# UBCMOCCA/mocca_envs

Hardware: AMD Instinct MI355X
Metric: env-steps/sec, Walker3DCustomEnv-v0 @ 4096 envs, 1/2/4/8 MI355X (higher is better)
Workload: dtype f32; 1 GPU; Walker3DCustomEnv-v0, 4096 envs/GPU, flat ground, U(-1,1) action tape, auto-reset; max_rows=48, max_contacts=12, envs_per_gpu=4096, parallelism=independent env shards x1, no collective, preroll_steps=6088

## Files before the change

### mocca_envs_amd/csrc/mocca_device.h

```cpp
#pragma once

#include <hip/hip_runtime.h>
#include <stdint.h>

#include "mocca_model.h"
#include "mocca_philox.h"
#include "topo_walker3d.h"
#include "topo_cassie.h"
#include "topo_walker2d.h"
#include "topo_crab2d.h"
#include "topo_laikago.h"

#define DI __device__ __forceinline__

#ifndef MOCCA_NS
#define MOCCA_NS mocca
#endif
#ifndef MOCCA_MAXR
#define MOCCA_MAXR 48
#endif
#ifndef MOCCA_COMPACT
#define MOCCA_COMPACT 0
#endif

// ... 82 lines not shown
  L_XL = L_V,
  L_MID = L_CAND + (MOCCA_MAX_PAIRS + 1) / 2,
  L_LGAP = L_GP,
  L_TOTAL = L_V + MAXR * MAXR + 28 + MOCCA_LDS_PAD,
#endif
};
static_assert(L_ABA_END <= L_TOTAL, "ABA view must fit");
static_assert(L_SV % 4 == 0 && SVS % 4 == 0 && SVS >= 16, "joint records live in the body records, 16-byte aligned");
static_assert(L_J + (MAXR + 1) * 28 <= L_TOTAL, "Jacobian rows (+ dummy) must fit the tail of the A region");
static_assert(L_J % 4 == 0 && L_V % 4 == 0 && L_RT % 4 == 0 && L_CT % 4 == 0, "16-byte alignment of broadcast rows");
static_assert(MAXR % 2 == 0 && 3 * MAXC <= MAXR, "friction rows sit on the top 2 MAXC lanes of the row range, odd lane = second tangent");
static_assert(L_PLANK + 12 * MOCCA_MAX_PLANKS <= L_V && L_Q0 + 16 <= L_V, "persistent region overflows into the two-view region");
#if MOCCA_COMPACT
static_assert(L_TOTAL * 4 <= 8192 || MOCCA_LDS_PAD > 0, "more than 8 KB of LDS per wave: fewer than 20 waves per CU (5 per SIMD)");
static_assert(L_J >= L_SV + 22 * SVS, "J rows are written while S, V, 1/D are still being read");
static_assert(L_CAND + (MOCCA_MAX_PAIRS + 1) / 2 <= L_ABA_END && L_RT + 264 <= L_GP, "frames, geom points and the candidate list live under the link inertias");
#else
static_assert(L_TOTAL * 4 <= 10240 || MOCCA_LDS_PAD > 0 || MAXR > 48, "more than 10 KB of LDS per wave: fewer than 16 waves per CU, the 4096-env batch no longer fits one round");
static_assert(MAXR != 48 || (L_ROWD == L_V + 848 && L_RT == L_V + 896 && L_M == L_V + 1160 && L_P == L_V + 1952 && L_ABA_END == L_V + 2084 && L_J == L_V + 960), "the product's layout is unchanged");
static_assert(COMPACT || L_CAND + (MOCCA_MAX_PAIRS + 1) / 2 <= L_TOTAL, "candidate list behind the ABA view");
static_assert(L_J >= L_RT, "J rows may be written while S, U, 1/D, the factor of IA0 and the contacts are still being read");
static_assert(L_LGAP + MAXR <= L_CT && L_J >= L_CT, "limit gaps: written after the collision pass, read before the first J row or A entry is stored");
#endif
#if MOCCA_COMPACT
static_assert(L_LGAP >= L_J + 28 * (MAXR + 1) && L_LGAP >= L_A + MAXR * MAXR && L_LGAP >= L_M && L_LGAP + MAXR <= L_TOTAL, "limit gaps: behind the solver view, in the dead link inertias");
#endif
static_assert(L_MID % 4 == 0 && L_MID >= L_CAND + (MOCCA_MAX_PAIRS + 1) / 2, "midpoint records: 16-byte aligned, behind the candidate list");
template <class T>
#ifdef MOCCA_NO_TRIM_1
constexpr bool MID_RECORDS = false;
#else
constexpr bool MID_RECORDS = T::NPAIR > 0 && 6 * T::NG <= GP_FLOATS && L_MID + 4 * T::NG <= (COMPACT ? (int)L_ABA_END : (int)L_TOTAL);
#endif

enum : int { C_BA = 0, C_BB = 1, C_SLOT = 2, C_P = 3, C_N = 6, C_DEPTH = 9, C_MU = 10, C_ERP = 11, C_CFM = 12, C_MA = 13, C_MB = 14 };

struct StepArgs {
  const MoccaModel* model;
  float* dyn;
  uint32_t* task;
  float* terrain;
  const float* act;
  float* obs;
  float* rew;
  uint8_t* done;
  int32_t* info;
  const uint8_t* mask;
  int n_envs;
  int obs_dim;
  int auto_reset;
  int eval_mode;
  int random_pose;
  int curriculum;
  int host_retarget;
  int env_offset;
  uint32_t seed_lo, seed_hi;
  const float* curriculum_v;
  const float* eval_mode_v;
  int random_reward;
  const float* gain_v;
  float gain;
  const int32_t* inj_touch;
  const int32_t* inj_target;
  const int32_t* inj_body;
  const float* tape;
  int tape_n;
  int32_t* dbg;
  const float* traj;
  int traj_n;
  double traj_tmax, traj_cstep;
  int prio;
  const float* hf;
  int hf_rows, hf_cols;
  float hf_scale;
  float* final_obs;
  int persist_warm;
  const int32_t* order;
  int pace;
  unsigned long long* pace_acc;
  float* ep_ret;
  float* ep_masks;
  float* ep_bad;
  void* ep_rec;
  float* ep_totals;
  uint32_t ep_serial;
  float* robot_state;
  const float* base_value;
  int32_t* hf_field;
  int hf_stride, hf_n_fields, hf_redraw;
};
constexpr int ROBOT_STATE_STRIDE = 64;

DI void wsync() {
  __builtin_amdgcn_fence(__ATOMIC_RELEASE, "wavefront");
  __builtin_amdgcn_wave_barrier();
  __builtin_amdgcn_fence(__ATOMIC_ACQUIRE, "wavefront");
}
DI float dot3(const float* a, const float* b) { return a[0] * b[0] + a[1] * b[1] + a[2] * b[2]; }
DI void cross3(const float* a, const float* b, float* o) {
  float x = a[1] * b[2] - a[2] * b[1], y = a[2] * b[0] - a[0] * b[2], z = a[0] * b[1] - a[1] * b[0];
  o[0] = x; o[1] = y; o[2] = z;
}
DI float dot6(const float* a, const float* b) {
  return a[0] * b[0] + a[1] * b[1] + a[2] * b[2] + a[3] * b[3] + a[4] * b[4] + a[5] * b[5];
}
DI void matvec3(const float* R, const float* x, float* o) {
  float a = R[0] * x[0] + R[1] * x[1] + R[2] * x[2];
  float b = R[3] * x[0] + R[4] * x[1] + R[5] * x[2];
  float c = R[6] * x[0] + R[7] * x[1] + R[8] * x[2];
  o[0] = a; o[1] = b; o[2] = c;
}
DI void matmul3(const float* A, const float* B, float* C) {
  float T[9];
#pragma unroll
  for (int i = 0; i < 3; ++i)
#pragma unroll
    for (int j = 0; j < 3; ++j) T[3 * i + j] = A[3 * i] * B[j] + A[3 * i + 1] * B[3 + j] + A[3 * i + 2] * B[6 + j];
#pragma unroll
  for (int i = 0; i < 9; ++i) C[i] = T[i];
}
DI void quat_to_mat(const float* q, float* R) {
  float x = q[0], y = q[1], z = q[2], w = q[3];
  R[0] = 1 - 2 * (y * y + z * z); R[1] = 2 * (x * y - z * w); R[2] = 2 * (x * z + y * w);
  R[3] = 2 * (x * y + z * w); R[4] = 1 - 2 * (x * x + z * z); R[5] = 2 * (y * z - x * w);
  R[6] = 2 * (x * z - y * w); R[7] = 2 * (y * z + x * w); R[8] = 1 - 2 * (x * x + y * y);
// ... 104 lines not shown
  v = fmaxf(v, dpp_mov<0x140>(v));
  return fmaxf(fmaxf(readlane(v, 0), readlane(v, 16)), fmaxf(readlane(v, 32), readlane(v, 48)));
}

DI float rng_uniform(uint32_t slo, uint32_t shi, uint32_t env, uint32_t episode, uint32_t d) {
  uint32_t o[4];
  philox4x32(d >> 2, episode, env, 0u, slo, shi, o);
  uint32_t w = (d & 3) == 0 ? o[0] : (d & 3) == 1 ? o[1] : (d & 3) == 2 ? o[2] : o[3];
  return (float)(w >> 8) * (1.0f / 16777216.0f);
}

template <bool INJECT>
DI float draw_u(const StepArgs& a, int env, int episode, int d) {
  if constexpr (INJECT) {
    if (a.tape) return d < a.tape_n ? a.tape[(size_t)(env - a.env_offset) * a.tape_n + d] : 0.5f;
  }
  return rng_uniform(a.seed_lo, a.seed_hi, (uint32_t)env, (uint32_t)episode, (uint32_t)d);
}

struct WalkConsts { float cl[3], inl[6], ms, jarm, jdamp; };
template <bool FULL>
DI void walk_consts(ModelP M, int b, WalkConsts& k) {
#pragma unroll
  for (int i = 0; i < 3; ++i) k.cl[i] = M->com[b][i];
#pragma unroll
  for (int i = 0; i < 6; ++i) k.inl[i] = 0.0f;
  k.ms = 0; k.jarm = 0; k.jdamp = 0;
  if (FULL) {
#pragma unroll
    for (int i = 0; i < 6; ++i) k.inl[i] = M->inertia[b][i];
    k.ms = M->mass[b]; k.jarm = M->jarm[b]; k.jdamp = M->jdamp[b];
  }
}
template <class T>
DI void walk_phase1(float* L, int lane, unsigned long long ppk) {
  static_assert(3 * (T::NB - 1) <= 63, "three lanes per body must fit the wave (lane 63 writes the base)");
  {
    const int g = (lane * 43) >> 7;
    const int ri = lane - 3 * g;
    const int bg = g + 1 < T::NB ? g + 1 : 0;
    const unsigned plo = (unsigned)__shfl((int)(unsigned)ppk, bg, 64), phi = (unsigned)__shfl((int)(unsigned)(ppk >> 32), bg, 64);
    const unsigned long long pk3 = ((unsigned long long)phi << 32) | plo;
    float Rb[9];
    {
      float q[4] = {L[L_BASE + 3], L[L_BASE + 4], L[L_BASE + 5], L[L_BASE + 6]};
      quat_to_mat(q, Rb);
    }
    float row[3] = {ri == 0 ? Rb[0] : ri == 1 ? Rb[3] : Rb[6], ri == 0 ? Rb[1] : ri == 1 ? Rb[4] : Rb[7], ri == 0 ? Rb[2] : ri == 1 ? Rb[5] : Rb[8]};
    float rr = 0.0f;
#pragma unroll
    for (int k = 0; k < T::MAXD; ++k) {
      const int j = (int)((pk3 >> (5 * k)) & 31ull);
      const float4* jr = reinterpret_cast<const float4*>(L + L_SV + SVS * j);
      const float4 r0 = jr[0], r1 = jr[1], r2 = jr[2];
      rr += row[0] * r2.y + row[1] * r2.z + row[2] * r2.w;
      const float n0 = row[0] * r0.x + row[1] * r0.w + row[2] * r1.z;
      const float n1 = row[0] * r0.y + row[1] * r1.x + row[2] * r1.w;
      const float n2 = row[0] * r0.z + row[1] * r1.y + row[2] * r2.x;
      row[0] = n0; row[1] = n1; row[2] = n2;
    }
    if (bg > 0) {
      const float4 r3 = reinterpret_cast<const float4*>(L + L_SV + SVS * bg)[3];
      *reinterpret_cast<float4*>(L + L_RT + 12 * bg + 4 * ri) = make_float4(row[0], row[1], row[2], rr);
      L[L_SV + SVS * bg + ri] = row[0] * r3.x + row[1] * r3.y + row[2] * r3.z;
    }
    if (lane == 63) {
#pragma unroll
      for (int i = 0; i < 3; ++i) *reinterpret_cast<float4*>(L + L_RT + 4 * i) = make_float4(Rb[3 * i], Rb[3 * i + 1], Rb[3 * i + 2], 0.0f);
    }
  }
}
template <class T, bool FULL>
DI void walk_phase2(ModelP M, float* L, int lane, int b, unsigned long long ppk, const WalkConsts& wk) {
  const float cl[3] = {wk.cl[0], wk.cl[1], wk.cl[2]};
  const float inl[6] = {wk.inl[0], wk.inl[1], wk.inl[2], wk.inl[3], wk.inl[4], wk.inl[5]};
  const float ms = wk.ms, jarm = wk.jarm, jdamp = wk.jdamp;
  float R[9], r[3], v[6], S[6] = {0, 0, 0, 0, 0, 0}, c[6] = {0, 0, 0, 0, 0, 0};
#pragma unroll
  for (int i = 0; i < 3; ++i) {
    const float4 t = *reinterpret_cast<const float4*>(L + L_RT + 12 * b + 4 * i);
    R[3 * i] = t.x; R[3 * i + 1] = t.y; R[3 * i + 2] = t.z; r[i] = t.w;
  }
  if (FULL) {
    if (lane >= 1 && lane < T::NB) {
      float a[3] = {L[L_SV + SVS * b], L[L_SV + SVS * b + 1], L[L_SV + SVS * b + 2]}, ra[3];
      cross3(r, a, ra);
#pragma unroll
      for (int i = 0; i < 3; ++i) { S[i] = a[i]; S[3 + i] = ra[i]; L[L_SV + SVS * b + 3 + i] = ra[i]; }
    }
    wsync();
#pragma unroll
    for (int k = 0; k < 3; ++k) { v[k] = L[L_BASE + 10 + k]; v[3 + k] = L[L_BASE + 7 + k]; }
#pragma unroll
    for (int k = 0; k < T::MAXD; ++k) {
      const int j = (int)((ppk >> (5 * k)) & 31ull);
      if (j != 0 && j != b) {
        const float qd = L[L_QD + j];
// ... 53 lines not shown
      p[0] -= cw[1] * fz; p[1] -= -cw[0] * fz; p[5] -= fz;
      {
        float om[3] = {v[0], v[1], v[2]}, Iom[3], wxc[3], F[3], cxF[3];
        float Iwf[9] = {Iw[0], Iw[1], Iw[2], Iw[1], Iw[4], Iw[5], Iw[2], Iw[5], Iw[8]};
        matvec3(Iwf, om, Iom);
        cross3(om, cw, wxc);
        float vc[3] = {v[3] + wxc[0], v[4] + wxc[1], v[5] + wxc[2]};
        const float kl = unif(M->lin_damp) * ms * (1.0f + __builtin_sqrtf(dot3(vc, vc)));
        const float ka = unif(M->ang_damp) * (1.0f + __builtin_sqrtf(dot3(om, om)));
#pragma unroll
        for (int i = 0; i < 3; ++i) F[i] = kl * vc[i];
        cross3(cw, F, cxF);
#pragma unroll
        for (int i = 0; i < 3; ++i) { p[i] += ka * Iom[i] + cxF[i]; p[3 + i] += F[i]; }
      }
#pragma unroll
      for (int i = 0; i < 6; ++i)
#pragma unroll
        for (int jx = 0; jx < 6; ++jx) L[L_M + 36 * b + 6 * i + jx] = I[sym(i, jx)];
#pragma unroll
      for (int i = 0; i < 6; ++i) L[L_P + 6 * b + i] = p[i];
      L[L_SV + SVS * b + SV_INVD] = jarm;
      L[L_SV + SVS * b + SV_UU] = L[L_TAU + b] - jdamp * L[L_QD + b];
    }
  }
}

template <class T, bool FULL>
DI void walk_kinematics(ModelP M, float* L, int lane, unsigned long long ppk) {
  asm volatile("" : "+v"(lane));
  const int b = lane < T::NB ? lane : 0;
  WalkConsts wk;
  walk_consts<FULL>(M, b, wk);
  walk_phase1<T>(L, lane, ppk);
  wsync();
  walk_phase2<T, FULL>(M, L, lane, b, ppk, wk);
}

DI void chol6_factor(const float* A, float* F) {
  float Lm[6][6];
#pragma unroll
  for (int j = 0; j < 6; ++j) {
    float s = A[sym(j, j)];
#pragma unroll
    for (int k = 0; k < j; ++k) s -= Lm[j][k] * Lm[j][k];
    const float id = rsq(s);
    F[sym(j, j)] = id;
#pragma unroll
    for (int i = j + 1; i < 6; ++i) {
      float t = A[sym(i, j)];
#pragma unroll
      for (int k = 0; k < j; ++k) t -= Lm[i][k] * Lm[j][k];
      Lm[i][j] = t * id;
      F[sym(i, j)] = Lm[i][j];
    }
  }
}
DI void chol6_solve(const float* F, const float* b, float* x) {
  float y[6];
#pragma unroll
  for (int j = 0; j < 6; ++j) {
    float t = b[j];
#pragma unroll
    for (int k = 0; k < j; ++k) t -= F[sym(j, k)] * y[k];
    y[j] = t * F[sym(j, j)];
  }
#pragma unroll
// ... 1172 lines not shown
    for (int i = 0; i < 6; ++i) { S[i] = L[L_SV + SVS * jj + i]; U[i] = L[L_SV + SVS * jj + SV_V + i]; }
    float jb = dot6(S, F);
    if (jj == jl) jb = sgn;
    jb = valid ? jb : 0.0f;
    const float uu = valid ? (k == T::MAXD - 1 ? jb : jb - dot6(S, pa)) : 0.0f;
#pragma unroll
    for (int i = 0; i < 6; ++i) pa[i] += U[i] * uu;
    if (valid) Jrow[5 + jj] = jb;
    w += jb * L[L_NU + 5 + jj];
    pu[k] = uu * L[L_SV + SVS * jj + SV_INVD];
    pin6(pa); pin1(pu[k]); pin1(w);
  }
  if (two_paths) {
    const int bq = bb >= 0 ? bb : 0;
    const unsigned long long pkb = ((unsigned long long)(unsigned)__shfl((int)(unsigned)(ppk >> 32), bq, 64) << 32) |
                                   (unsigned long long)(unsigned)__shfl((int)(unsigned)ppk, bq, 64);
#pragma unroll
    for (int k = T::MAXD - 1; k >= 0; --k) {
      const int j = (int)((pkb >> (5 * k)) & 31ull);
      const bool valid = j != 0;
      const int jj = j;
      float S[6], U[6];
#pragma unroll
      for (int i = 0; i < 6; ++i) { S[i] = L[L_SV + SVS * jj + i]; U[i] = L[L_SV + SVS * jj + SV_V + i]; }
      const float jb = valid ? -dot6(S, F2) : 0.0f;
      const float uu = valid ? (k == T::MAXD - 1 ? jb : jb - dot6(S, pb)) : 0.0f;
#pragma unroll
      for (int i = 0; i < 6; ++i) pb[i] += U[i] * uu;
      if (valid) Jrow[5 + jj] += jb;
      w += jb * L[L_NU + 5 + jj];
      pub[k] = uu * L[L_SV + SVS * jj + SV_INVD];
      pin6(pb); pin1(pub[k]); pin1(w);
    }
  } else {
#pragma unroll
    for (int k = 0; k < T::MAXD; ++k) pub[k] = 0.0f;
  }
  STAMP(19);
  int l2off = 0;
  asm volatile("" : "+v"(l2off));
  l2off &= ~3;
  const float* L2 = L + l2off;
  float a0[6];
  {
    float rhs[6];
#pragma unroll
    for (int i = 0; i < 6; ++i) {
      const float jb = F[i] * sa - F2[i] * sb;
      Jrow[i] = jb;
      w += jb * L[L_NU + i];
      rhs[i] = jb - (pa[i] + pb[i]);
    }
    chol6_solve(Afac, rhs, a0);
#pragma unroll
    for (int i = 0; i < 6; ++i) X[i] = a0[i];
  }
  {
    float acc[T::NB][6];
#pragma unroll
    for (int i = 0; i < 6; ++i) acc[0][i] = a0[i];
#pragma unroll
    for (int b = 1; b < T::NB; ++b) {
      const int p = T::parent(b);
      float S[6], U[6];
#pragma unroll
      for (int i = 0; i < 6; ++i) { S[i] = L2[L_SV + SVS * b + i]; U[i] = L2[L_SV + SVS * b + SV_V + i]; }
      const int dpos = T::depth(b) - 1;
      float ub = __uint_as_float(__float_as_uint(pu[dpos]) & (unsigned)__builtin_amdgcn_sbfe((int)ma, b, 1));
      if (two_paths) ub += __uint_as_float(__float_as_uint(pub[dpos]) & (unsigned)__builtin_amdgcn_sbfe((int)mb, b, 1));
      const float qdd = ub - dot6(U, acc[p]);
      X[5 + b] = qdd;
#pragma unroll
      for (int i = 0; i < 6; ++i) acc[b][i] = acc[p][i] + S[i] * qdd;
      pin6(acc[b]); pin1(X[5 + b]);
    }
  }
  STAMP(6);
  wsync();
  const int lc = has_row ? dense : MAXR - 1;
  float diag;
  bool on_mfma = false;
  if constexpr (T::NCLOS == 0 && MATRIX_PIPE) on_mfma = nr >= MOCCA_DELASSUS_MFMA_MIN && nr <= DELASSUS_MFMA_ROWS && !(wave_flags & 2);
  if (on_mfma) {
    diag = delassus_mfma<T>(L, X, has_row ? dense : 0, has_row, nr, lane);
  } else {
    float av[MAXR / 2 + 1];
    const int cc = has_row ? dense : 0, tmax = nr >> 1;
    delassus_dots<T, 0>(L, X, 28 * cc, 28 * nr, tmax, av);
    diag = has_row ? av[0] : 1.0f;
    wsync();
    if (has_row) delassus_store<0>(L, cc, nr, tmax, av);
  }
  const float invdiag = diag + cfm > 1e-12f ? rcp(diag + cfm) : 0.0f;
  wsync();
  STAMP(7);
  if (__ballot(lam != 0.0f) != 0ull) {
    int rr = nl + NFIX;
    const int rend = nl + NFIX + nc;
#pragma unroll 1
    for (; rr + 2 <= rend; rr += 2) {
      const float g0 = L[L_A + MAXR * rr + lc], g1 = L[L_A + MAXR * rr + MAXR + lc];
      w += g0 * readlane(lam, rr); w += g1 * readlane(lam, rr + 1);
    }
    if (rr < rend) w += L[L_A + MAXR * rr + lc] * readlane(lam, rr);
  }
  STAMP(20);
  const int iters = uni(M->n_iters);
// ... 108 lines not shown
      const float k = hdt * sinc;
      dq[0] = om[0] * k; dq[1] = om[1] * k; dq[2] = om[2] * k;
    } else {
      const float wn = sqrtf(dot3(om, om)), sn = sinf(wn * hdt) / wn;
      dq[0] = om[0] * sn; dq[1] = om[1] * sn; dq[2] = om[2] * sn; dq[3] = cosf(wn * hdt);
    }
    const float q0 = L[L_BASE + 3], q1 = L[L_BASE + 4], q2 = L[L_BASE + 5], q3 = L[L_BASE + 6];
    float nq[4];
    nq[0] = dq[3] * q0 + dq[0] * q3 + dq[1] * q2 - dq[2] * q1;
    nq[1] = dq[3] * q1 - dq[0] * q2 + dq[1] * q3 + dq[2] * q0;
    nq[2] = dq[3] * q2 + dq[0] * q1 - dq[1] * q0 + dq[2] * q3;
    nq[3] = dq[3] * q3 - dq[0] * q0 - dq[1] * q1 - dq[2] * q2;
    const float nn = rsq(nq[0] * nq[0] + nq[1] * nq[1] + nq[2] * nq[2] + nq[3] * nq[3]);
#pragma unroll
    for (int i = 0; i < 4; ++i) L[L_BASE + 3 + i] = nq[i] * nn;
  }
  wsync();
}

DI void fast_sincos(float q, float* s, float* c) {
  const float k = rintf(q * 0.636619772f);
  float r = fmaf(-k, 1.57079601e+00f, q);
  r = fmaf(-k, 3.13916473e-07f, r);
  r = fmaf(-k, 5.39030253e-15f, r);
  const float r2 = r * r;
  const float sr = r + r * r2 * (-1.0f / 6 + r2 * (1.0f / 120 + r2 * (-1.0f / 5040 + r2 * (1.0f / 362880))));
  const float cr = 1.0f + r2 * (-0.5f + r2 * (1.0f / 24 + r2 * (-1.0f / 720 + r2 * (1.0f / 40320 + r2 * (-1.0f / 3628800)))));
  const int qd = (int)k & 3;
  const float ss = (qd & 1) ? cr : sr, cc = (qd & 1) ? sr : cr;
  *s = (qd & 2) ? -ss : ss;
  *c = ((qd + 1) & 2) ? -cc : cc;
}

template <class T>
DI void stage_joints(ModelP M, float* L, int lane) {
  if (lane < T::NB) {
    const int j = lane;
    float s, cq;
    fast_sincos(L[L_Q + j], &s, &cq);
    const float t = 1.0f - cq;
    float ax[3], jr[9], Rq[9], Tl[9];
#pragma unroll
    for (int i = 0; i < 3; ++i) ax[i] = M->jaxis[j][i];
#pragma unroll
    for (int i = 0; i < 9; ++i) jr[i] = M->jrot[j][i];
    Rq[0] = cq + t * ax[0] * ax[0];          Rq[1] = t * ax[0] * ax[1] - s * ax[2];   Rq[2] = t * ax[0] * ax[2] + s * ax[1];
    Rq[3] = t * ax[0] * ax[1] + s * ax[2];   Rq[4] = cq + t * ax[1] * ax[1];          Rq[5] = t * ax[1] * ax[2] - s * ax[0];
    Rq[6] = t * ax[0] * ax[2] - s * ax[1];   Rq[7] = t * ax[1] * ax[2] + s * ax[0];   Rq[8] = cq + t * ax[2] * ax[2];
    matmul3(jr, Rq, Tl);
    float4* rec = reinterpret_cast<float4*>(L + L_SV + SVS * j);
    rec[0] = make_float4(Tl[0], Tl[1], Tl[2], Tl[3]);
    rec[1] = make_float4(Tl[4], Tl[5], Tl[6], Tl[7]);
    rec[2] = make_float4(Tl[8], M->jpos[j][0], M->jpos[j][1], M->jpos[j][2]);
    rec[3] = make_float4(ax[0], ax[1], ax[2], L[L_QD + j]);
  }
  wsync();
}

template <class T, int TASK>
DI ContactFlags substep(ModelP M, float* L, int lane, const float* ter, int next_step_index,
                        unsigned long long ppk, int32_t* dbg, int prio, int& rows_out,
                        const HeightFieldArgs hfa = HeightFieldArgs{nullptr, 0, 0, 0.0f}, int sidx = 0, int nsub = 1, int* cover_out = nullptr) {
  const int per0 = 64 + MOCCA_PACE_ROWUNIT * rows_out, done0 = sidx * per0, total = nsub * per0;
  STAMP(30);
  stage_joints<T>(M, L, lane);
  STAMP(29);
  int nc = 0, nc_wanted = 0;
  float Afac[21] = {0, 0, 0, 0, 0, 0, 0, 0, 0, 0, 0, 0, 0, 0, 0, 0, 0, 0, 0, 0, 0};
  ContactFlags fl = {0, 0, 0, 0, 0, 0, 0, 0, 0};
  if constexpr (COMPACT) {
    static_assert(!COMPACT || T::NCLOS == 0, "closure rows read the body frames after the ABA: not in the compact layout");
    int wl = lane;
    asm volatile("" : "+v"(wl));
    walk_phase1<T>(L, wl, ppk);
    wsync();
    STAMP(0);
    geom_points<T>(M, L, lane);
    wsync();
    STAMP(15);
#ifndef MOCCA_SKIP_COLLIDE
    fl = collide<T, TASK>(M, L, lane, ter, next_step_index, &nc, dbg, &nc_wanted, hfa, cover_out);
#endif
    wsync();
    const int wb = wl < T::NB ? wl : 0;
    WalkConsts wk;
    walk_consts<true>(M, wb, wk);
    walk_phase2<T, true>(M, L, wl, wb, ppk, wk);
// ... 226 lines not shown
      dx = sg * (mx < d1 ? mx : d1);
    }
    float x = 0, y = 0, z = 0, rx = 0, ry = 0, rz = 0;
#pragma unroll 1
    for (int k = 0; k < N; ++k) {
      rx += readlane(dx, k); ry += readlane(dy, k); rz += readlane(dz, k);
      if (lane == k) { x = rx; y = ry; z = rz; }
    }
    if (lane < N) {
      ter[6 * i] = x; ter[6 * i + 1] = y; ter[6 * i + 2] = z; ter[6 * i + 3] = phi; ter[6 * i + 4] = xt; ter[6 * i + 5] = yt;
    }
    if (lane == 0) { ter[120] = 0.0f; ter[121] = 1.0f; ter[122] = 2.0f; ter[123] = 3.0f; }
  }
  wsync();
}

DI int live_curriculum(const StepArgs& a, int env) {
  if (a.curriculum_v) { const int c = (int)a.curriculum_v[env]; return c < 0 ? 0 : (c > 9 ? 9 : c); }
  return a.curriculum;
}
DI bool live_eval_mode(const StepArgs& a, int env) { return a.eval_mode_v ? a.eval_mode_v[env] != 0.0f : a.eval_mode != 0; }

template <class T>
DI float reset_base_pose(ModelP M, float* L, int lane) {
  if (lane == 0) {
#pragma unroll
    for (int i = 0; i < 3; ++i) { L[L_BASE + i] = M->init_pos[i]; L[L_BASE + 7 + i] = M->init_vel[i]; L[L_BASE + 10 + i] = 0; }
#pragma unroll
    for (int i = 0; i < 4; ++i) L[L_BASE + 3 + i] = M->init_quat[i];
  }
  if (lane < MOCCA_MAX_SLOTS) L[L_WARM + lane] = 0.0f;
  wsync();
  const float z0 = L[L_BASE + 2];
  stage_joints<T>(M, L, lane);
  walk_kinematics<T, false>(M, L, lane, T::path_packed(lane < T::NB ? lane : 0));
  wsync();
  return z0;
}

template <class T, int TASK, bool INJECT = false>
DI void reset_env(const StepArgs& a, ModelP M, float* L, float* ter, int env, int lane, TaskRegs& t,
                  float* obs) {
  const int ep = t.episode + 1, cur = t.cur;
  const float sfc[4] = {t.fc0, t.fc1, t.fc2, t.fc3};
  const int snsi = t.nsi, scover = t.cover;
  t = TaskRegs{};
  t.episode = ep;
  if (TASK == MOCCA_TASK_WALKER3D_STEPPER && (M->task_flags & MOCCA_TASKF_STALE_RESET_CONTACTS)) {
    t.fc0 = sfc[0]; t.fc1 = sfc[1]; t.fc2 = sfc[2]; t.fc3 = sfc[3];
    const int npl = M->n_planks;
    int reached = cover_targets(scover, snsi, npl, 0) | cover_targets(scover, snsi, npl, 1);
    if constexpr (T::NFEET > 2) reached |= cover_targets(scover, snsi, npl, 2) | cover_targets(scover, snsi, npl, 3);
    if (reached) t.trc = 1;
  }
  t.cur = TASK == MOCCA_TASK_WALKER3D_STEPPER ? live_curriculum(a, env - a.env_offset) : cur;
  t.gain = a.gain_v ? a.gain_v[env - a.env_offset] : a.gain;
  if (TASK == MOCCA_TASK_WALKER3D_CUSTOM) {
    randomize_target<INJECT>(a, env, t, live_eval_mode(a, env - a.env_offset));
    float sa, ca;
    fast_sincos(t.angle, &sa, &ca);
    t.wt[0] = t.dist * ca;
    t.wt[1] = t.dist * sa;
    t.wt[2] = 1.0f;
  } else if (TASK == MOCCA_TASK_WALKER3D_STEPPER) {
    t.gain = M->gain_cur[0] + (M->gain_cur[1] - M->gain_cur[0]) * t.cur / 9;
  }
  t.mirrored = draw_u<INJECT>(a, env, t.episode, t.draw) < 0.5f;
// ... 237 lines not shown
```

### mocca_envs_amd/csrc/mocca_kernels.h

```cpp
#pragma once
#include <hip/hip_runtime.h>

#include "mocca.h"
#include "mocca_device.h"

namespace MOCCA_NS {

#ifndef MOCCA_WAVES_PER_EU
#define MOCCA_WAVES_PER_EU 4
#endif

DI void flush_obs(const float* L, float* dst, int lane, int obs_dim) {
#pragma unroll 1
  for (int k = lane; k < obs_dim; k += 64) dst[k] = L[L_OBS + k];
}
DI void keep_terminal_obs(const StepArgs& a, const float* L, int env, int lane) {
  wsync();
  if (a.final_obs) flush_obs(L, a.final_obs + (size_t)env * a.obs_dim, lane, a.obs_dim);
  wsync();
}

template <class T>
DI void keep_robot_state(const StepArgs& a, const float* L, int env, int lane) {
  static_assert(ROBOT_OBS<T> <= 64 && ROBOT_OBS<T> <= ROBOT_STATE_STRIDE, "one store per lane");
// ... 155 lines not shown
  if (cur_idx != t.nsi) calc_potential(M, L, t, ro, &dist, &cd, &sd);
  float rew;
  if (!a.random_reward) {
    rew = progress - energy + step_bonus + bonus + tall - posture - joints;
  } else {
    const float terms[8] = {progress, -energy, step_bonus, bonus, 0.0f, tall, -posture, -joints};
    rew = 0.0f;
#pragma unroll
    for (int k = 0; k < 8; ++k) {
      float w;
      if (a.random_reward == 1) {
        w = 0.8f + 0.4f * draw_u<INJECT>(a, env + a.env_offset, t.episode, t.draw + k);
        if (lane == 0) tk[MOCCA_TW_REWARD_WEIGHTS + k] = __float_as_uint(w);
      } else {
        w = __uint_as_float(tk[MOCCA_TW_REWARD_WEIGHTS + k]);
      }
      rew += w * terms[k];
    }
    if (a.random_reward == 1) t.draw += 8;
  }
  t.cover = cover;
  return {rew, t.nsi};
}

template <class T>
DI StepResult cassie_step(const StepArgs& __restrict__ a, ModelP M, float* L, uint32_t* tk, int lane, unsigned long long ppk, TaskRegs& __restrict__ t,
                          float* obs) {
  t.istep += M->n_llc;
  float jv = 0.0f;
  if (lane < M->n_ordered) {
    jv = (L[L_Q + M->ordered_body[lane]] - L[L_Q0 + lane]) / M->control_dt;
    tk[MOCCA_TW_JVEL + lane] = __float_as_uint(jv);
  }
  stage_joints<T>(M, L, lane);
  walk_kinematics<T, false>(M, L, lane, ppk);
  wsync();
  t.t += 1;
  const CassieState cs = cassie_state(M, L, lane, t.initz);
  const float old = t.linpot;
  t.linpot = cassie_potential(M, L);
  const float alive = cs.height > M->alive_height ? 2.0f : -1.0f;
  if (!cs.finite || alive < 0.0f) t.done = 1;
  float rew = alive + (t.linpot - old);
  float phase = 0.0f;
  if (M->cassie_mode != MOCCA_CASSIE_PLAIN) {
    const int f1 = traj_frame(a, M, t.istep, &phase);
    rew = cassie_mocap_reward(a, M, L, lane, cs, jv, f1);
  }
  cassie_observe(M, L, lane, cs, t.initz, jv, phase, obs);
  return {rew, 0};
}

template <class T, int TASK, bool INJECT = false>
__global__ __launch_bounds__(64, MOCCA_WAVES_PER_EU) void mocca_step_kernel(StepArgs a) {
  __shared__ float L[L_TOTAL];
  const int lane = threadIdx.x;
  if ((int)blockIdx.x >= a.n_envs) return;
  const int env = a.order ? uni(a.order[blockIdx.x]) : (int)blockIdx.x;
  ModelP M = (ModelP)a.model;
  float* st = a.dyn + (size_t)env * DYN_STRIDE;
  uint32_t* tk = a.task + (size_t)env * MOCCA_TASK_WORDS;
  float* ter = TASK == MOCCA_TASK_WALKER3D_STEPPER ? a.terrain + (size_t)env * TERRAIN_STRIDE : nullptr;
  float* obs_out = a.obs + (size_t)env * a.obs_dim;
  float* obs = L + L_OBS;
  int32_t* dbg = a.dbg ? a.dbg + (size_t)env * MOCCA_DEBUG_WORDS : nullptr;

  const bool warm_ld = INJECT || uni(__float_as_int(M->warmstart)) != 0, warm_st = warm_ld || a.persist_warm != 0;
  if (dbg && lane == 0) { dbg[16] = 0; dbg[17] = 0; dbg[18] = 0; }
  load_dyn(st, L, lane, T::NJ, T::NSLOT, warm_ld);
  pace_start(a, L, lane, INJECT ? 0 : a.pace);
  if (lane == 0) L[L_KEEPWARM] = __int_as_float((warm_st ? 1 : 0) | ((a.prio & PRIO_DELASSUS_VALU) ? 2 : 0));
  const unsigned long long ppk = T::path_packed(lane < T::NB ? lane : 0);
  ContactFlags fl = {0, 0, 0, 0, 0, 0, 0, 0, 0};
  int cover = 0;
  if constexpr (TASK == MOCCA_TASK_CASSIE) {
    const int no = M->n_ordered, nctl = M->n_ctrl, mode = M->cassie_mode;
    float target = 0.0f;
    if (lane < nctl) {
      float base = M->ctrl_base[lane];
      if (mode != MOCCA_CASSIE_PLAIN) {
        const int f0 = traj_frame(a, M, (int)tk[MOCCA_TW_ISTEP]);
        base = (lane < nctl - 2 && M->residual_control) ? a.traj[(size_t)f0 * MOCCA_TRAJ_STRIDE + M->ctrl_oidx[lane]] : 0.0f;
      }
      target = base + (lane < nctl - 2 ? a.act[(size_t)env * (nctl - 2) + lane] : 0.0f);
    }
    if (lane < no) {
      L[L_JVEL + lane] = __uint_as_float(tk[MOCCA_TW_JVEL + lane]);
      L[L_Q0 + lane] = L[L_Q + M->ordered_body[lane]];
    }
    if (lane < MOCCA_MAX_BODIES) L[L_TAU + lane] = 0.0f;
    if (lane == 0) { L[L_Q] = 0.0f; L[L_QD] = 0.0f; }
    wsync();
    const int nllc = INJECT ? 0 : M->n_llc;
    int last_rows = uni((int)tk[MOCCA_TW_LAST_ROWS]);
    if (!INJECT && a.pace == 0) set_issue_priority(last_rows, a.prio);
#pragma unroll 1
    for (int it = 0; it < nllc; ++it) {
      ModelP Ms = M;
      int ln = lane;
      unsigned long long pk = ppk;
      asm volatile("" : "+s"(Ms), "+v"(ln), "+v"(pk));
      if (ln < no) {
        const float al = Ms->jvel_alpha;
        L[L_JVEL + ln] = (1.0f - al) * L[L_JVEL + ln] + al * L[L_QD + Ms->ordered_body[ln]];
      }
      wsync();
      if (ln < nctl) {
        const int b = Ms->ctrl_body[ln];
        const float perr = target - L[L_Q + b];
        float verr = -L[L_JVEL + Ms->ctrl_oidx[ln]];
        verr = verr < -5.0f ? -5.0f : (verr > 5.0f ? 5.0f : verr);
        const float tq = Ms->ctrl_kp[ln] * perr + Ms->ctrl_kd[ln] * verr, lim = Ms->torque_limit[b];
        L[L_TAU + b] = tq < -lim ? -lim : (tq > lim ? lim : tq);
      }
      wsync();
      substep<T, TASK>(Ms, L, ln, nullptr, 0, pk, dbg, a.prio, last_rows, HeightFieldArgs{nullptr, 0, 0, 0.0f}, it, nllc);
    }
    if (!INJECT && lane == 0) tk[MOCCA_TW_LAST_ROWS] = (uint32_t)last_rows;
  } else {
    {
      const float applied_gain = __uint_as_float(tk[MOCCA_TW_APPLIED_GAIN]);
      if (lane < T::NJ) {
        const float act_raw = a.act[(size_t)env * T::NJ + lane];
        const float c = act_raw < -1.0f ? -1.0f : (act_raw > 1.0f ? 1.0f : act_raw);
        L[L_TAU + 1 + lane] = M->gain[lane + 1] * applied_gain * c;
      }
    }
    if (lane == 0) { L[L_TAU] = 0.0f; L[L_Q] = 0.0f; L[L_QD] = 0.0f; }
    wsync();

    STAMP(28);
    if constexpr (TASK == MOCCA_TASK_WALKER3D_STEPPER) stage_planks(M, L, lane, ter);
    const int nsub = INJECT ? 0 : M->n_substeps;
    const int nsi0 = TASK == MOCCA_TASK_WALKER3D_STEPPER ? (int)tk[MOCCA_TW_NEXT_STEP_INDEX] : 0;
    int last_rows = uni((int)tk[MOCCA_TW_LAST_ROWS]);
    if (!INJECT && a.pace == 0) set_issue_priority(last_rows, a.prio);
    const float* hfp = a.hf;
    if constexpr (TASK == MOCCA_TASK_WALKER3D_PLANNER) hfp = env_heightfield(a, env);
#pragma unroll 1
    for (int s = 0; s < nsub; ++s) {
      ModelP Ms = M;
      int ln = lane;
      unsigned long long pk = ppk;
      asm volatile("" : "+s"(Ms), "+v"(ln), "+v"(pk));
      fl = substep<T, TASK>(Ms, L, ln, ter, nsi0, pk, dbg, a.prio, last_rows, HeightFieldArgs{hfp, a.hf_rows, a.hf_cols, a.hf_scale}, s, nsub, &cover);
    }
    if constexpr (INJECT) {
      const int32_t* tc = a.inj_touch + (size_t)env * T::NFEET;
      fl.touch0 = tc[0] != 0; fl.touch1 = tc[1] != 0;
      if constexpr (T::NFEET > 2) { fl.touch2 = tc[2] != 0; fl.touch3 = tc[3] != 0; }
      if (a.inj_target) {
        const int32_t* tg = a.inj_target + (size_t)env * T::NFEET;
        const int npl = TASK == MOCCA_TASK_WALKER3D_STEPPER ? M->n_planks : 1;
#pragma unroll
        for (int f = 0; f < T::NFEET; ++f)
          if (tg[f] == 1 || tg[f] == 2) cover |= 1 << (4 * f + (nsi0 + tg[f] - 1) % npl);
        fl.target0 = tg[0] == 1; fl.target1 = tg[1] == 1;
        if constexpr (T::NFEET > 2) { fl.target2 = tg[2] == 1; fl.target3 = tg[3] == 1; }
      }
      if (a.inj_body) fl.body_touch = a.inj_body[env] != 0;
    }
    if (!INJECT && lane == 0) tk[MOCCA_TW_LAST_ROWS] = (uint32_t)last_rows;
    STAMP(27);
  }
  TaskRegs t = load_task<T, TASK>(tk);
  const float ep_ret0 = a.ep_ret ? a.ep_ret[env] : 0.0f;
  StepResult r;
  if constexpr (TASK == MOCCA_TASK_CASSIE) r = cassie_step<T>(a, M, L, tk, lane, ppk, t, obs);
  else {
    const float act_raw = lane < T::NJ ? a.act[(size_t)env * T::NJ + lane] : 0.0f;
    {
      int lo = lane;
      asm volatile("" : "+v"(lo));
      stage_joints<T>(M, L, lo);
      walk_kinematics<T, false>(M, L, lo, ppk);
    }
    wsync();
    t.t += 1;
    if constexpr (TASK == MOCCA_TASK_WALKER3D_PLANNER) r = planner_step<T>(M, L, lane, t, fl, obs, a.base_value ? a.base_value + env : nullptr);
    else if constexpr (TASK == MOCCA_TASK_WALKER3D_CUSTOM) r = custom_step<T, INJECT>(a, M, L, env, lane, t, fl, act_raw, obs);
    else r = stepper_step<T, INJECT>(a, M, L, ter, tk, env, lane, t, fl, cover, act_raw, obs);
    t.prevx = L[L_BASE];
  }
  const int timeout = t.t >= M->max_episode_steps;
  const int dflag = (t.done ? 1 : 0) | (timeout ? 2 : 0);
  if (lane == 0) {
    a.rew[env] = r.rew;
    a.done[env] = (uint8_t)dflag;
    if (a.info) a.info[env] = r.info;
    if (a.ep_ret) monitor_emit(a, env, ep_ret0, r.rew, dflag, t.t, r.info);
  }
  STAMP(26);
  if (a.auto_reset && dflag) {
    keep_terminal_obs(a, L, env, lane);
    reset_task<T, TASK, INJECT>(a, M, L, ter, tk, env + a.env_offset, lane, t, obs);
  }
  wsync();
  flush_obs(L, obs_out, lane, a.obs_dim);
  if constexpr (TASK == MOCCA_TASK_WALKER3D_PLANNER) keep_robot_state<T>(a, L, env, lane);
  store_dyn(st, L, lane, T::NJ, T::NSLOT, (uni(__float_as_int(L[L_KEEPWARM])) & 1) != 0);
  if (lane == 0) store_task<T, TASK, true>(tk, t);
  if (!INJECT) pace_finish(a, L, lane, a.pace);
  STAMP(25);
#ifdef MOCCA_STAMPS
  if (lane == 0 && blockIdx.x < STAMP_WAVES) g_stamps[blockIdx.x * STAMP_SLOTS + 24] = (unsigned long long)(a.auto_reset && dflag);
#endif
}

template <class T, int TASK, bool INJECT = false>
__global__ __launch_bounds__(64) void mocca_reset_kernel(StepArgs a) {
  __shared__ float L[L_TOTAL];
  const int env = blockIdx.x, lane = threadIdx.x;
  if (env >= a.n_envs) return;
  if (a.mask && !a.mask[env]) return;
  ModelP M = (ModelP)a.model;
  float* st = a.dyn + (size_t)env * DYN_STRIDE;
  uint32_t* tk = a.task + (size_t)env * MOCCA_TASK_WORDS;
  float* ter = TASK == MOCCA_TASK_WALKER3D_STEPPER ? a.terrain + (size_t)env * TERRAIN_STRIDE : nullptr;
  TaskRegs t = load_task<T, TASK, true>(tk);
  if (lane == 0) { L[L_Q] = 0.0f; L[L_QD] = 0.0f; if (a.ep_ret) a.ep_ret[env] = 0.0f; }
  reset_task<T, TASK, INJECT>(a, M, L, ter, tk, env + a.env_offset, lane, t, L + L_OBS);
  wsync();
  flush_obs(L, a.obs + (size_t)env * a.obs_dim, lane, a.obs_dim);
  if constexpr (TASK == MOCCA_TASK_WALKER3D_PLANNER) keep_robot_state<T>(a, L, env, lane);
  store_dyn(st, L, lane, T::NJ, T::NSLOT);
  if (lane == 0) store_task<T, TASK, true>(tk, t);
}

template <class T, int TASK>
__global__ __launch_bounds__(64) void mocca_observe_kernel(StepArgs a) {
  __shared__ float L[L_TOTAL];
  const int env = blockIdx.x, lane = threadIdx.x;
  if (env >= a.n_envs) return;
  ModelP M = (ModelP)a.model;
  const float* st = a.dyn + (size_t)env * DYN_STRIDE;
  uint32_t* tk = a.task + (size_t)env * MOCCA_TASK_WORDS;
  const float* ter = TASK == MOCCA_TASK_WALKER3D_STEPPER ? a.terrain + (size_t)env * TERRAIN_STRIDE : nullptr;
  float* obs = L + L_OBS;
  load_dyn(st, L, lane, T::NJ, T::NSLOT);
  TaskRegs t = load_task<T, TASK>(tk);
  if (lane == 0) { L[L_Q] = 0.0f; L[L_QD] = 0.0f; }
  wsync();
  stage_joints<T>(M, L, lane);
  walk_kinematics<T, false>(M, L, lane, T::path_packed(lane < T::NB ? lane : 0));
  wsync();
  if constexpr (TASK == MOCCA_TASK_CASSIE) {
    const CassieState cs = cassie_state(M, L, lane, t.initz);
    float phase = 0.0f;
    if (M->cassie_mode != MOCCA_CASSIE_PLAIN) traj_frame(a, M, t.istep, &phase);
    cassie_observe(M, L, lane, cs, t.initz, lane < MOCCA_MAX_CTRL ? __uint_as_float(tk[MOCCA_TW_JVEL + lane]) : 0.0f, phase, obs);
    t.linpot = cassie_potential(M, L);
  } else {
    RobotObs ro = robot_obs<T>(M, L, lane, t.fc0, t.fc1, obs, t.fc2, t.fc3);
    float dist, cd, sd;
    if (TASK == MOCCA_TASK_WALKER3D_CUSTOM || TASK == MOCCA_TASK_WALKER3D_PLANNER) {
      calc_potential(M, L, t, ro, &dist, &cd, &sd);
      if (lane == 0) softsign_tail(sd, cd, obs + ROBOT_OBS<T>);
    } else {
      delta_to_k_targets(M, L, ter, t, ro, lane, obs + ROBOT_OBS<T>);
      calc_potential(M, L, t, ro, &dist, &cd, &sd);
    }
    t.prevx = L[L_BASE];
  }
  wsync();
  flush_obs(L, a.obs + (size_t)env * a.obs_dim, lane, a.obs_dim);
  if constexpr (TASK == MOCCA_TASK_WALKER3D_PLANNER) keep_robot_state<T>(a, L, env, lane);
  if (lane == 0) store_task<T, TASK>(tk, t);
}


enum { TOPO_WALKER3D = 0, TOPO_CASSIE = 1, TOPO_WALKER2D = 2, TOPO_CRAB2D = 3, TOPO_LAIKAGO = 4,
       TOPO_WALKER3D_MASSIVE = 5, TOPO_CASSIE_MASSIVE = 6  };
template <template <class, int> class Launcher, class... Args>
static void dispatch(int topo, int task_id, Args... args) {
  if (topo == TOPO_CASSIE || topo == TOPO_CASSIE_MASSIVE) {
    if constexpr (!COMPACT) {
// ... 23 lines not shown
```

Before: 42.47 million env-steps/s.

## Trim dead axis staging, leaf accelerations, and reload kernel args late

Several independent trims land together. Joint-axis records and the world-axis write are skipped when kinematics runs without full dynamics. Leaf bodies skip the spatial acceleration update in the forward pass, and the zero-fill of the unused second-path buffer is dropped. Kernel arguments are also re-read from the kernarg segment after the substep loop, for selected configurations including the non-compact Walker3D custom task, so they need not stay live in scalar registers throughout. The aim is less LDS traffic, fewer ALU ops and lower register pressure, at the cost of extra scalar loads and more complex code.

```diff
diff --git a/mocca_envs_amd/csrc/mocca_device.h b/mocca_envs_amd/csrc/mocca_device.h
--- a/mocca_envs_amd/csrc/mocca_device.h
+++ b/mocca_envs_amd/csrc/mocca_device.h
@@ -138,6 +138,12 @@
 #else
 constexpr bool MID_RECORDS = T::NPAIR > 0 && 6 * T::NG <= GP_FLOATS && L_MID + 4 * T::NG <= (COMPACT ? (int)L_ABA_END : (int)L_TOTAL);
 #endif
+template <class T>
+constexpr bool has_child(int b) {
+  for (int k = 0; k < T::MAXCH; ++k)
+    if (T::cchild(b, k) >= 0) return true;
+  return false;
+}
 
 enum : int { C_BA = 0, C_BB = 1, C_SLOT = 2, C_P = 3, C_N = 6, C_DEPTH = 9, C_MU = 10, C_ERP = 11, C_CFM = 12, C_MA = 13, C_MB = 14 };
 
@@ -197,6 +203,22 @@
 };
 constexpr int ROBOT_STATE_STRIDE = 64;
 
+DI void read_kernargs(StepArgs& la) {
+  auto p = __builtin_amdgcn_kernarg_segment_ptr();
+  asm volatile("" : "+s"(p));
+  __builtin_memcpy(&la, p, sizeof(StepArgs));
+}
+template <bool LATE>
+DI void late_args(StepArgs& la) {
+  if constexpr (LATE) read_kernargs(la);
+}
+template <class T, int TASK, bool INJECT>
+#ifdef MOCCA_NO_TRIM_7
+constexpr bool LATE_ARGS = false;
+#else
+constexpr bool LATE_ARGS = INJECT || MAXR > 48 || !__is_base_of(TopoWalker3D, T) || (!COMPACT && TASK == MOCCA_TASK_WALKER3D_CUSTOM);
+#endif
+
 DI void wsync() {
   __builtin_amdgcn_fence(__ATOMIC_RELEASE, "wavefront");
   __builtin_amdgcn_wave_barrier();
@@ -367,8 +389,14 @@
     k.ms = M->mass[b]; k.jarm = M->jarm[b]; k.jdamp = M->jdamp[b];
   }
 }
-template <class T>
+#ifdef MOCCA_NO_TRIM_6
+template <class T, bool AXES_ = true>
 DI void walk_phase1(float* L, int lane, unsigned long long ppk) {
+  constexpr bool AXES = true;
+#else
+template <class T, bool AXES = true>
+DI void walk_phase1(float* L, int lane, unsigned long long ppk) {
+#endif
   static_assert(3 * (T::NB - 1) <= 63, "three lanes per body must fit the wave (lane 63 writes the base)");
   {
     const int g = (lane * 43) >> 7;
@@ -395,9 +423,9 @@
       row[0] = n0; row[1] = n1; row[2] = n2;
     }
     if (bg > 0) {
-      const float4 r3 = reinterpret_cast<const float4*>(L + L_SV + SVS * bg)[3];
+      const float4 r3 = AXES ? reinterpret_cast<const float4*>(L + L_SV + SVS * bg)[3] : make_float4(0.0f, 0.0f, 0.0f, 0.0f);
       *reinterpret_cast<float4*>(L + L_RT + 12 * bg + 4 * ri) = make_float4(row[0], row[1], row[2], rr);
-      L[L_SV + SVS * bg + ri] = row[0] * r3.x + row[1] * r3.y + row[2] * r3.z;
+      if constexpr (AXES) L[L_SV + SVS * bg + ri] = row[0] * r3.x + row[1] * r3.y + row[2] * r3.z;
     }
     if (lane == 63) {
 #pragma unroll
@@ -517,7 +545,7 @@
   const int b = lane < T::NB ? lane : 0;
   WalkConsts wk;
   walk_consts<FULL>(M, b, wk);
-  walk_phase1<T>(L, lane, ppk);
+  walk_phase1<T, FULL>(L, lane, ppk);
   wsync();
   walk_phase2<T, FULL>(M, L, lane, b, ppk, wk);
 }
@@ -1756,10 +1784,13 @@
       pub[k] = uu * L[L_SV + SVS * jj + SV_INVD];
       pin6(pb); pin1(pub[k]); pin1(w);
     }
-  } else {
+  }
+#ifdef MOCCA_NO_TRIM_5
+  else {
 #pragma unroll
     for (int k = 0; k < T::MAXD; ++k) pub[k] = 0.0f;
   }
+#endif
   STAMP(19);
   int l2off = 0;
   asm volatile("" : "+v"(l2off));
@@ -1786,17 +1817,26 @@
 #pragma unroll
     for (int b = 1; b < T::NB; ++b) {
       const int p = T::parent(b);
-      float S[6], U[6];
-#pragma unroll
-      for (int i = 0; i < 6; ++i) { S[i] = L2[L_SV + SVS * b + i]; U[i] = L2[L_SV + SVS * b + SV_V + i]; }
+#ifdef MOCCA_NO_TRIM_4
+      constexpr bool inner = true;
+#else
+      const bool inner = has_child<T>(b);
+#endif
+      float U[6];
+#pragma unroll
+      for (int i = 0; i < 6; ++i) U[i] = L2[L_SV + SVS * b + SV_V + i];
       const int dpos = T::depth(b) - 1;
       float ub = __uint_as_float(__float_as_uint(pu[dpos]) & (unsigned)__builtin_amdgcn_sbfe((int)ma, b, 1));
       if (two_paths) ub += __uint_as_float(__float_as_uint(pub[dpos]) & (unsigned)__builtin_amdgcn_sbfe((int)mb, b, 1));
       const float qdd = ub - dot6(U, acc[p]);
       X[5 + b] = qdd;
-#pragma unroll
-      for (int i = 0; i < 6; ++i) acc[b][i] = acc[p][i] + S[i] * qdd;
-      pin6(acc[b]); pin1(X[5 + b]);
+      if (inner) {
+        float S[6];
+#pragma unroll
+        for (int i = 0; i < 6; ++i) { S[i] = L2[L_SV + SVS * b + i]; acc[b][i] = acc[p][i] + S[i] * qdd; }
+        pin6(acc[b]);
+      }
+      pin1(X[5 + b]);
     }
   }
   STAMP(6);
@@ -1971,8 +2011,14 @@
   *c = ((qd + 1) & 2) ? -cc : cc;
 }
 
-template <class T>
+#ifdef MOCCA_NO_TRIM_6
+template <class T, bool AXES_ = true>
 DI void stage_joints(ModelP M, float* L, int lane) {
+  constexpr bool AXES = true;
+#else
+template <class T, bool AXES = true>
+DI void stage_joints(ModelP M, float* L, int lane) {
+#endif
   if (lane < T::NB) {
     const int j = lane;
     float s, cq;
@@ -1991,7 +2037,7 @@
     rec[0] = make_float4(Tl[0], Tl[1], Tl[2], Tl[3]);
     rec[1] = make_float4(Tl[4], Tl[5], Tl[6], Tl[7]);
     rec[2] = make_float4(Tl[8], M->jpos[j][0], M->jpos[j][1], M->jpos[j][2]);
-    rec[3] = make_float4(ax[0], ax[1], ax[2], L[L_QD + j]);
+    if constexpr (AXES) rec[3] = make_float4(ax[0], ax[1], ax[2], L[L_QD + j]);
   }
   wsync();
 }
@@ -2284,7 +2330,7 @@
   if (lane < MOCCA_MAX_SLOTS) L[L_WARM + lane] = 0.0f;
   wsync();
   const float z0 = L[L_BASE + 2];
-  stage_joints<T>(M, L, lane);
+  stage_joints<T, false>(M, L, lane);
   walk_kinematics<T, false>(M, L, lane, T::path_packed(lane < T::NB ? lane : 0));
   wsync();
   return z0;
diff --git a/mocca_envs_amd/csrc/mocca_kernels.h b/mocca_envs_amd/csrc/mocca_kernels.h
--- a/mocca_envs_amd/csrc/mocca_kernels.h
+++ b/mocca_envs_amd/csrc/mocca_kernels.h
@@ -211,7 +211,7 @@
     jv = (L[L_Q + M->ordered_body[lane]] - L[L_Q0 + lane]) / M->control_dt;
     tk[MOCCA_TW_JVEL + lane] = __float_as_uint(jv);
   }
-  stage_joints<T>(M, L, lane);
+  stage_joints<T, false>(M, L, lane);
   walk_kinematics<T, false>(M, L, lane, ppk);
   wsync();
   t.t += 1;
@@ -252,6 +252,9 @@
   const unsigned long long ppk = T::path_packed(lane < T::NB ? lane : 0);
   ContactFlags fl = {0, 0, 0, 0, 0, 0, 0, 0, 0};
   int cover = 0;
+  constexpr bool LATE = LATE_ARGS<T, TASK, INJECT>;
+  StepArgs late, late_reset;
+  const StepArgs& al = LATE ? late : a;
   if constexpr (TASK == MOCCA_TASK_CASSIE) {
     const int no = M->n_ordered, nctl = M->n_ctrl, mode = M->cassie_mode;
     float target = 0.0f;
@@ -295,6 +298,7 @@
       wsync();
       substep<T, TASK>(Ms, L, ln, nullptr, 0, pk, dbg, a.prio, last_rows, HeightFieldArgs{nullptr, 0, 0, 0.0f}, it, nllc);
     }
+    late_args<LATE>(late);
     if (!INJECT && lane == 0) tk[MOCCA_TW_LAST_ROWS] = (uint32_t)last_rows;
   } else {
     {
@@ -324,12 +328,13 @@
       asm volatile("" : "+s"(Ms), "+v"(ln), "+v"(pk));
       fl = substep<T, TASK>(Ms, L, ln, ter, nsi0, pk, dbg, a.prio, last_rows, HeightFieldArgs{hfp, a.hf_rows, a.hf_cols, a.hf_scale}, s, nsub, &cover);
     }
+    late_args<LATE>(late);
     if constexpr (INJECT) {
-      const int32_t* tc = a.inj_touch + (size_t)env * T::NFEET;
+      const int32_t* tc = al.inj_touch + (size_t)env * T::NFEET;
       fl.touch0 = tc[0] != 0; fl.touch1 = tc[1] != 0;
       if constexpr (T::NFEET > 2) { fl.touch2 = tc[2] != 0; fl.touch3 = tc[3] != 0; }
-      if (a.inj_target) {
-        const int32_t* tg = a.inj_target + (size_t)env * T::NFEET;
+      if (al.inj_target) {
+        const int32_t* tg = al.inj_target + (size_t)env * T::NFEET;
         const int npl = TASK == MOCCA_TASK_WALKER3D_STEPPER ? M->n_planks : 1;
 #pragma unroll
         for (int f = 0; f < T::NFEET; ++f)
@@ -337,52 +342,55 @@
         fl.target0 = tg[0] == 1; fl.target1 = tg[1] == 1;
         if constexpr (T::NFEET > 2) { fl.target2 = tg[2] == 1; fl.target3 = tg[3] == 1; }
       }
-      if (a.inj_body) fl.body_touch = a.inj_body[env] != 0;
+      if (al.inj_body) fl.body_touch = al.inj_body[env] != 0;
     }
     if (!INJECT && lane == 0) tk[MOCCA_TW_LAST_ROWS] = (uint32_t)last_rows;
     STAMP(27);
   }
   TaskRegs t = load_task<T, TASK>(tk);
-  const float ep_ret0 = a.ep_ret ? a.ep_ret[env] : 0.0f;
+  const float ep_ret0 = al.ep_ret ? al.ep_ret[env] : 0.0f;
   StepResult r;
-  if constexpr (TASK == MOCCA_TASK_CASSIE) r = cassie_step<T>(a, M, L, tk, lane, ppk, t, obs);
+  if constexpr (TASK == MOCCA_TASK_CASSIE) r = cassie_step<T>(al, M, L, tk, lane, ppk, t, obs);
   else {
-    const float act_raw = lane < T::NJ ? a.act[(size_t)env * T::NJ + lane] : 0.0f;
+    const float act_raw = lane < T::NJ ? al.act[(size_t)env * T::NJ + lane] : 0.0f;
     {
       int lo = lane;
       asm volatile("" : "+v"(lo));
-      stage_joints<T>(M, L, lo);
+      stage_joints<T, false>(M, L, lo);
       walk_kinematics<T, false>(M, L, lo, ppk);
     }
     wsync();
     t.t += 1;
-    if constexpr (TASK == MOCCA_TASK_WALKER3D_PLANNER) r = planner_step<T>(M, L, lane, t, fl, obs, a.base_value ? a.base_value + env : nullptr);
-    else if constexpr (TASK == MOCCA_TASK_WALKER3D_CUSTOM) r = custom_step<T, INJECT>(a, M, L, env, lane, t, fl, act_raw, obs);
-    else r = stepper_step<T, INJECT>(a, M, L, ter, tk, env, lane, t, fl, cover, act_raw, obs);
+    if constexpr (TASK == MOCCA_TASK_WALKER3D_PLANNER) r = planner_step<T>(M, L, lane, t, fl, obs, al.base_value ? al.base_value + env : nullptr);
+    else if constexpr (TASK == MOCCA_TASK_WALKER3D_CUSTOM) r = custom_step<T, INJECT>(al, M, L, env, lane, t, fl, act_raw, obs);
+    else r = stepper_step<T, INJECT>(al, M, L, ter, tk, env, lane, t, fl, cover, act_raw, obs);
     t.prevx = L[L_BASE];
   }
   const int timeout = t.t >= M->max_episode_steps;
   const int dflag = (t.done ? 1 : 0) | (timeout ? 2 : 0);
   if (lane == 0) {
-    a.rew[env] = r.rew;
-    a.done[env] = (uint8_t)dflag;
-    if (a.info) a.info[env] = r.info;
-    if (a.ep_ret) monitor_emit(a, env, ep_ret0, r.rew, dflag, t.t, r.info);
+    al.rew[env] = r.rew;
+    al.done[env] = (uint8_t)dflag;
+    if (al.info) al.info[env] = r.info;
+    if (al.ep_ret) monitor_emit(al, env, ep_ret0, r.rew, dflag, t.t, r.info);
   }
   STAMP(26);
-  if (a.auto_reset && dflag) {
-    keep_terminal_obs(a, L, env, lane);
-    reset_task<T, TASK, INJECT>(a, M, L, ter, tk, env + a.env_offset, lane, t, obs);
-  }
-  wsync();
-  flush_obs(L, obs_out, lane, a.obs_dim);
-  if constexpr (TASK == MOCCA_TASK_WALKER3D_PLANNER) keep_robot_state<T>(a, L, env, lane);
+  if (al.auto_reset && dflag) {
+    late_args<LATE>(late_reset);
+    const StepArgs& ar = LATE ? late_reset : a;
+    keep_terminal_obs(ar, L, env, lane);
+    reset_task<T, TASK, INJECT>(ar, M, L, ter, tk, env + ar.env_offset, lane, t, obs);
+  }
+  wsync();
+  late_args<LATE>(late);
+  flush_obs(L, LATE ? al.obs + (size_t)env * al.obs_dim : obs_out, lane, al.obs_dim);
+  if constexpr (TASK == MOCCA_TASK_WALKER3D_PLANNER) keep_robot_state<T>(al, L, env, lane);
   store_dyn(st, L, lane, T::NJ, T::NSLOT, (uni(__float_as_int(L[L_KEEPWARM])) & 1) != 0);
   if (lane == 0) store_task<T, TASK, true>(tk, t);
-  if (!INJECT) pace_finish(a, L, lane, a.pace);
+  if (!INJECT) pace_finish(al, L, lane, al.pace);
   STAMP(25);
 #ifdef MOCCA_STAMPS
-  if (lane == 0 && blockIdx.x < STAMP_WAVES) g_stamps[blockIdx.x * STAMP_SLOTS + 24] = (unsigned long long)(a.auto_reset && dflag);
+  if (lane == 0 && blockIdx.x < STAMP_WAVES) g_stamps[blockIdx.x * STAMP_SLOTS + 24] = (unsigned long long)(al.auto_reset && dflag);
 #endif
 }
 
@@ -420,7 +428,7 @@
   TaskRegs t = load_task<T, TASK>(tk);
   if (lane == 0) { L[L_Q] = 0.0f; L[L_QD] = 0.0f; }
   wsync();
-  stage_joints<T>(M, L, lane);
+  stage_joints<T, false>(M, L, lane);
   walk_kinematics<T, false>(M, L, lane, T::path_packed(lane < T::NB ? lane : 0));
   wsync();
   if constexpr (TASK == MOCCA_TASK_CASSIE) {
```

Measured after the change: 43.04 million env-steps/s, median of 6. +1.3%, better.
